# alshai/rowbowt

Hardware: AMD Instinct MI355X
Metric: reads/s (100 bp, count+locate) (higher is better)
Workload: dtype u32/u64

## Files before the change

### rowbowt_amd/csrc/k_runs.hip

```cpp
#include <type_traits>

#include "rbg_runs2_device.hpp"
#include "rbg_jump.h"

namespace rbg {
namespace {

struct PackedBits {
    const uint4 *__restrict__ cp;
    uint4 w;
    uint32_t widx, navail;
    uint64_t sr;
    __device__ __forceinline__ uint32_t next_word() {
        if (widx == 4) { w = *cp++; widx = 0; }
        const uint32_t v = w.x;
        w.x = w.y; w.y = w.z; w.z = w.w;
        ++widx;
        return v;
    }
    __device__ __forceinline__ uint32_t take(uint32_t nb) {
        if (navail < nb) { sr |= static_cast<uint64_t>(next_word()) << navail; navail += 32; }
        const uint32_t v = static_cast<uint32_t>(sr & ((uint64_t(1) << nb) - 1));
        sr >>= nb;
        navail -= nb;
        return v;
    }
};

struct JumpLoad {
    const uint4 *__restrict__ tab;
    __device__ __forceinline__ void operator()(uint64_t b, uint32_t s, uint32_t kw[4], uint32_t vw[4]) const {
        const uint4 *sl = tab + (4 * b + 2 * s);
        const uint4 k = sl[0], v = sl[1];
        kw[0] = k.x; kw[1] = k.y; kw[2] = k.z; kw[3] = k.w;
        vw[0] = v.x; vw[1] = v.y; vw[2] = v.z; vw[3] = v.w;
    }
};

template <typename P, bool TOEHOLD, bool PACKED = false, bool STATS = false, bool GLDS = false, bool STAGE = false>
__global__ __launch_bounds__(512, STATS ? 2 : 4) void k_find_range_runs(const DevIndex ix, const void *__restrict__ src_a,
                                                        const void *__restrict__ src_b, const uint64_t N,
                                                        uint64_t *__restrict__ lo_out, uint64_t *__restrict__ hi_out,
                                                        uint64_t *__restrict__ ss_out, unsigned long long *__restrict__ stats,
                                                        const uint32_t *__restrict__ sel, const uint32_t *__restrict__ nsel) {
    const uint64_t Neff = sel ? static_cast<uint64_t>(*nsel) : N;
    const uint8_t *__restrict__ seqs = static_cast<const uint8_t *>(src_a);
    const uint64_t *__restrict__ off = static_cast<const uint64_t *>(src_b);
    const uint4 *__restrict__ chunks = static_cast<const uint4 *>(src_a);
    const uint2 *__restrict__ meta = static_cast<const uint2 *>(src_b);
    __shared__ uint8_t s_lut[256];
    __shared__ uint8_t s_lut2[256];
    __shared__ uint8_t s_mslot[4];
    __shared__ __align__(16) unsigned char s_tile[GLDS ? 8 * kTileBytes : 16];
    __shared__ uint32_t s_codes[STAGE ? 8 * kStageWords * 64 : 1];
    for (int t = threadIdx.x; t < 256; t += blockDim.x) {
        s_lut[t] = ix.lut[t];
        s_lut2[t] = ix.nmajor ? ix.lut2[t] : 0xFFu;
    }
    RBG_RUN_SEARCH2_SHARED;
    const RunSearch2<P> S2 = stage_run_search2<P>(ix, s_tab_first, s_ent2, s_dir2, s_rec2, s_dyn);
    const uint32_t *tab_first = s_tab_first;
    lds_byte *tile = (lds_byte *)s_tile + (GLDS ? (threadIdx.x >> 6) * kTileBytes : 0u);
    if (PACKED || STAGE) {
        for (int t = threadIdx.x; t < 256; t += blockDim.x)
            if (s_lut2[t] != 0xFFu) s_mslot[s_lut2[t] & 3u] = s_lut[t];
        __syncthreads();
    }
    const uint32_t D = ix.run_ksteps, DMASK = ix.run_depth_mask | 1u;
    const uint32_t M = ix.nmajor;
    const uint32_t lane = threadIdx.x & (kWave - 1);
    lds_u32 *codes = (lds_u32 *)s_codes + (STAGE ? (threadIdx.x >> 6) * (kStageWords * 64u) + lane : 0u);
    const StageTab stage_tab{ix.stage_code[0], ix.stage_code[1], ix.stage_byte[0], ix.stage_byte[1], ix.stage_shift};
    const bool stage_on = STAGE && ix.stage_ok != 0 && M == 4;

    unsigned long long c_occ = 0, c_reads = 0;
    uint32_t c_matched = 0;
    unsigned long long st[kStatSearchN] = {0, 0, 0, 0, 0, 0, 0, 0};
    const uint64_t stride = static_cast<uint64_t>(gridDim.x) * blockDim.x;
    const uint64_t wave_first = static_cast<uint64_t>(blockIdx.x) * blockDim.x + (threadIdx.x & ~(kWave - 1));
    for (uint64_t base = wave_first; base < Neff; base += stride) {
        bool valid = base + lane < Neff;
        const uint64_t i = (sel && valid) ? static_cast<uint64_t>(sel[base + lane]) : base + lane;
        uint64_t beg = 0, p = 0;
        PackedBits bs{chunks, make_uint4(0, 0, 0, 0), 4u, 0u, 0ull};
        if (PACKED) {
            if (valid) {
                const uint2 mt = meta[i];
                if (mt.y & 0x80000000u) valid = false;
                else { p = mt.y; bs.cp = chunks + mt.x; }
            }
        } else if (valid) { beg = off[i]; p = off[i + 1]; }
        bool staged = false;
        if constexpr (STAGE && !PACKED) {
            if (stage_on && __ballot(valid && p - beg > kStageCap) == 0) {
                uint32_t nch = 0;
                const bool bad = valid && stage_read(reinterpret_cast<const uint4 *>(seqs), beg, p, stage_tab, codes, nch);
                if (STATS) st[kStChunks] += nch;
                staged = __ballot(bad) == 0;
                if (staged) { p -= beg; beg = 0; }
                else if (STATS) st[kStChunks] -= nch;
            }
        }
        auto walk = [&](auto staged_tag) __attribute__((always_inline)) {
            constexpr bool STAGED = decltype(staged_tag)::value;
            const uint64_t p_end = p;
            uint64_t p_min = p;
            const uint32_t m32 = static_cast<uint32_t>(p);
            uint64_t lo = 0, hi = ix.n - 1;
            uint64_t k = TOEHOLD ? ix.last_run_sample : 0;
            bool alive = valid;
            bool pend = false;
            uint32_t pend_d = 0, pend_rec = 0;
            uint64_t pend_e = 0;
            ByteCursor rd{reinterpret_cast<const uint4 *>(seqs), ~uint64_t(0), make_uint4(0, 0, 0, 0)};
            bool jumped = false;
            if constexpr (STAGED && sizeof(P) == 4) {
                if (valid && ix.jump && m32 >= ix.jump_k) {
                    JumpKey key{{codes[0], codes[64], codes[128], codes[192]}};
                    jump_key_mask(key, ix.jump_k);
                    uint32_t v[3] = {0, 0, 0}, nbk = 0;
                    if (jump_probe(JumpLoad{static_cast<const uint4 *>(ix.jump)}, ix.jump_buckets, key, v, nbk)) {
                        lo = v[0]; hi = v[1];
                        if (TOEHOLD) k = v[2] == 0xFFFFFFFFu ? ~uint64_t(0) : static_cast<uint64_t>(v[2]);
                        p -= ix.jump_k;
                        jumped = true;
                        if (STATS) st[kStSymbols] += ix.jump_k;
                    }
                    if (STATS) st[kStFtab] += nbk;
                }
            }
            if (!jumped && valid && ix.ftab_k && p - beg >= ix.ftab_k) {
                uint64_t idx = 0;
                bool all_major = true;
                PackedBits probe = bs;
                if constexpr (STAGED) {
                    const uint32_t w0 = codes[0];
                    idx = ix.ftab_k >= 16u ? w0 : (w0 & ((1u << (2u * ix.ftab_k)) - 1u));
                } else if (PACKED) {
                    idx = probe.take(2 * ix.ftab_k);
                } else {
                    uint64_t pw = 1;
                    for (uint32_t t = 1; t <= ix.ftab_k; ++t) {
                        const uint32_t mm = s_lut2[rd.at(p - t)];
                        all_major = all_major && mm != 0xFFu;
                        idx += (mm & 3u) * pw;
                        pw *= M;
                    }
                }
                uint64_t flo, fhi2, fk;
                if (STATS) { if (!STAGED) p_min = p - ix.ftab_k; if (all_major) st[kStFtab] += 1; }
                if (all_major && ftab_lookup<P>(ix, idx, flo, fhi2, fk)) {
                    if (PACKED) bs = probe;
                    lo = flo; hi = fhi2;
                    if (TOEHOLD) k = fk;
                    p -= ix.ftab_k;
                    if (STATS) st[kStSymbols] += ix.ftab_k;
                    if (hi < lo) { alive = false; p = beg; }
                }
            }
            struct Pick { uint32_t d, adv, rec; bool ok; };
            auto pick_at = [&](const uint64_t pp) __attribute__((always_inline)) -> Pick {
                Pick s{0u, 1u, 0u, true};
                if constexpr (STAGED) {
                    s.adv = pp < D ? static_cast<uint32_t>(pp) : D;
                    s.adv = 32u - static_cast<uint32_t>(__clz(DMASK & ((2u << (s.adv - 1)) - 1u)));
                    const uint32_t t0 = m32 - static_cast<uint32_t>(pp);
                    const lds_u32 *cw = codes + (t0 >> 4) * 64u;
                    const uint32_t v = __builtin_amdgcn_alignbit(cw[64], cw[0], (t0 & 15u) * 2u) & ((1u << (2u * s.adv)) - 1u);
                    s.rec = run_record(tab_first, s.adv, s.adv == 1 ? static_cast<uint32_t>(s_mslot[v]) : v);
                    s.d = s.adv - 1;
                } else if (PACKED) {
                    s.adv = pp < D ? static_cast<uint32_t>(pp) : D;
                    s.adv = 32u - static_cast<uint32_t>(__clz(DMASK & ((2u << (s.adv - 1)) - 1u)));
                    const uint32_t v = bs.take(2 * s.adv);
                    s.rec = run_record(tab_first, s.adv, s.adv == 1 ? static_cast<uint32_t>(s_mslot[v]) : v);
                    s.d = s.adv - 1;
                } else {
                    const uint64_t q = pp - 1;
                    const uint32_t c = rd.at(q);
                    if (STATS && q < p_min) p_min = q;
                    const uint32_t m0 = s_lut2[c];
                    uint32_t acc = m0;
                    if (m0 != 0xFFu) {
                        uint32_t pw = M, run_acc = m0;
    #pragma unroll 1
                        for (uint32_t t = 1; t < static_cast<uint32_t>(kMaxRunDepth); ++t) {
                            if (t >= D || q < beg + t) break;
                            const uint32_t mm = s_lut2[rd.at(q - t)];
                            if (STATS && q - t < p_min) p_min = q - t;
                            if (mm == 0xFFu) break;
                            run_acc += mm * pw;
                            pw *= M;
                            if ((DMASK >> t) & 1u) { s.adv = t + 1; acc = run_acc; }
                        }
                    }
                    if (s.adv == 1) {
                        const uint32_t slot = s_lut[c];
                        if (slot == 0xFFu || slot >= static_cast<uint32_t>(kLdsSyms)) s.ok = false;
                        else s.rec = run_record(tab_first, 1u, slot);
                    } else {
                        s.d = s.adv - 1;
                        s.rec = run_record(tab_first, s.adv, acc);
                    }
                }
                return s;
            };
            constexpr bool AHEAD = !PACKED || STAGED;
            Pick cur{0u, 1u, 0u, false};
            RunHot Rcur{0, 0};
            if (AHEAD && alive && p > beg) {
                cur = pick_at(p);
                if (cur.ok) Rcur = load_run_tab<P>(S2, cur.d, cur.rec);
            }
            while (__ballot(alive && p > beg)) {
                bool stepping = alive && p > beg;
                if (!AHEAD && stepping) {
                    cur = pick_at(p);
                    if (cur.ok) Rcur = load_run_tab<P>(S2, cur.d, cur.rec);
                }
                if (stepping && !cur.ok) { alive = false; stepping = false; }
                const uint32_t d = cur.d, adv = cur.adv, rec = cur.rec;
                const RunHot R = Rcur;
                const uint64_t p_next = p - adv;
                if (AHEAD && stepping && p_next > beg) {
                    cur = pick_at(p_next);
                    if (cur.ok) Rcur = load_run_tab<P>(S2, cur.d, cur.rec);
                }
                RunStep r;
                lane_lf2_quad<P, STATS, false, GLDS>(S2, stepping, d, rec, R, lo, hi + 1, r, st, tile);
                if (stepping) {
                    if (STATS) st[kStSymbols] += adv;
                    const uint64_t c_inside = r.c_upto - r.c_before;
                    if (c_inside == 0) {
                        alive = false;
                    } else {
                        if (TOEHOLD) {
                            if (r.inside) k = k - adv;
                            else { pend = true; pend_d = d; pend_rec = rec; pend_e = r.samp_e; k = 0; }
                        }
                        lo = r.F + r.c_before;
                        hi = lo + c_inside - 1;
                        p = p_next;
                    }
                }
            }
            if (TOEHOLD && alive && pend) {
                k += run_step_sample2<P>(ix, S2, pend_d, pend_rec, pend_e);
                if (STATS) st[kStResample] += 1;
            }
            if (STATS && !PACKED && !STAGED && p_end > p_min) st[kStChunks] += ((p_end - 1) >> 4) - (p_min >> 4) + 1;
            if (STATS && PACKED && valid) st[kStChunks] += (p_end + 63) >> 6;
            if (!alive) { lo = 1; hi = 0; k = 0; }
            if (valid) {
                lo_out[i] = lo;
                hi_out[i] = hi;
                if (TOEHOLD) ss_out[i] = k;
                c_reads += 1;
                if (alive) { c_matched += 1; c_occ += hi - lo + 1; }
            }
        };
        if (STAGE && staged) walk(std::integral_constant<bool, STAGE>{}); else walk(std::false_type{});
    }
    c_reads = wave_sum(c_reads);
    const unsigned long long w_matched = wave_sum(static_cast<unsigned long long>(c_matched));
    c_occ = wave_sum(c_occ);
    if (lane == 0 && c_reads) {
        atomicAdd(&ix.counters[0], c_reads);
        if (w_matched) atomicAdd(&ix.counters[1], w_matched);
        if (c_occ) atomicAdd(&ix.counters[2], c_occ);
    }
    if (STATS) {
#pragma unroll
        for (int t = 0; t < kStatSearchN; ++t) {
            const unsigned long long v = wave_sum(st[t]);
            if (lane == 0 && v) atomicAdd(&stats[t], v);
        }
    }
}

template <typename P> struct ChunkR { static constexpr int v = 8; };
__device__ __forceinline__ uint64_t locus_toehold_r(const DevIndex &ix, const uint64_t key, const uint64_t *__restrict__ k, const uint64_t i) {
    if (key == ~uint64_t(0)) return k[i];
    const uint32_t low = ix.order_lowbits, db = ix.order_dbits;
    const uint64_t doc = (key >> low) & ((uint64_t(1) << db) - 1u);
    return ix.order_docs[doc] + (((key >> (db + low)) << low) | (key & ((uint64_t(1) << low) - 1u)));
}

template <typename P, typename OUT = uint64_t, bool STATS = false, bool SUB = false, bool HI8 = false>
__global__ __launch_bounds__(256, 4) void k_locate_fill_runs2(const DevIndex ix, const uint64_t *__restrict__ lo,
                                                          const uint64_t *__restrict__ hi, const uint64_t *__restrict__ k,
                                                          const uint64_t N, const uint64_t max_hits,
                                                          const uint64_t *__restrict__ loc_off, OUT *__restrict__ locs,
                                                          const uint64_t *__restrict__ sub, const uint32_t *__restrict__ order,
                                                          const uint64_t *__restrict__ skeys, unsigned long long *__restrict__ stats) {
    constexpr int kChunkR = ChunkR<P>::v;
    constexpr bool RING = true;
    using Stage = ChainStage<P, kChunkR, SUB, RING, HI8>;
    __shared__ Stage S;
    const uint64_t out_elem0 = reinterpret_cast<uintptr_t>(locs) / sizeof(OUT);
    const int wv = threadIdx.x >> 6, lane = threadIdx.x & (kWave - 1);
    unsigned long long c_locs = 0;
    unsigned long long st_phi = 0, st_ent = 0, st_chains = 0;
    const uint64_t n = ix.n;
    const uint64_t stride = static_cast<uint64_t>(gridDim.x) * blockDim.x;
    for (uint64_t base = static_cast<uint64_t>(blockIdx.x) * blockDim.x + wv * kWave; base < N; base += stride) {
        const uint64_t j = base + lane;
        uint64_t i = j;
        if (order && j < N) i = order[j];
        uint64_t occ = 0, k1 = 0, dst = 0;
        if (i < N && j < N) {
            dst = loc_off[i];
            if (skeys) {
                if (ix.order_docs) k1 = locus_toehold_r(ix, skeys[j], k, i);
                else if (sizeof(P) == 4) { const uint32_t k32 = reinterpret_cast<const uint32_t *>(skeys)[j]; k1 = k32 == 0xFFFFFFFFu ? k[i] : k32; }
                else k1 = skeys[j];
                occ = loc_off[i + 1] - dst;
            } else {
                const uint64_t l = lo[i], h = hi[i];
                occ = h >= l ? h - l + 1 : 0;
                if (occ > max_hits) occ = max_hits;
                k1 = k[i];
            }
        }
        const uint64_t minus = (SUB && i < N && j < N) ? sub[i] : 0;
        const uint32_t a = (RING && occ) ? static_cast<uint32_t>((out_elem0 + dst) & static_cast<uint64_t>(kChunkR - 1)) : 0u;
        S.dst[wv][lane] = dst - a;
        if (SUB) S.minus[wv][lane] = minus;
        const bool off_text = Stage::kSentinel && k1 >= n;
        if (off_text && occ) locs[dst] = static_cast<OUT>(k1 - minus);
        c_locs += occ;
        if (STATS && occ) st_chains += 1;
        uint64_t wmax = occ + a;
#pragma unroll
        for (int o = kWave / 2; o > 0; o >>= 1) {
            const uint64_t other = __shfl_xor(wmax, o, kWave);
            wmax = other > wmax ? other : wmax;
        }
        for (uint64_t t0 = 0; t0 < wmax; t0 += kChunkR) {
            const uint32_t cnt = chain_round_count<kChunkR>(occ, t0);
            S.bounds[wv][lane] = chain_window_bounds<kChunkR>(occ, a, t0);
#pragma unroll 1
            for (int e = 0; e < kChunkR; ++e) {
                const bool mine = static_cast<uint32_t>(e) < cnt;
                if (mine && (e || t0)) {
                    uint64_t s;
                    if (k1 >= n) {
                        s = (ix.phi_last_base + (k1 - ix.phi_last_pos)) % n;
                    } else {
                        bool found;
                        uint64_t val;
                        uint32_t ents, rounds;
                        lane_phi<P>(ix, k1, found, val, ents, rounds);
                        if (STATS) { st_phi += 1; st_ent += ents + 7u * rounds; }
                        s = found ? val : ix.phi_last_base + k1 + 1;
                        if (s >= n) s -= n;
                    }
                    k1 = s;
                }
                if (mine) chain_put(S, wv, lane, a + static_cast<uint32_t>(t0) + e, k1, e == 0 && t0 == 0 && off_text);
            }
            wave_lds_sync();
            chain_flush(S, wv, lane, t0, locs);
            wave_lds_sync();
        }
        wave_lds_sync();
    }
    c_locs = wave_sum(c_locs);
    if (lane == 0 && c_locs) atomicAdd(&ix.counters[3], c_locs);
    if (STATS) {
        st_phi = wave_sum(st_phi);
        st_ent = wave_sum(st_ent);
        st_chains = wave_sum(st_chains);
        if (lane == 0) {
            if (st_phi) atomicAdd(&stats[kLsPhiSteps], st_phi);
            if (st_ent) atomicAdd(&stats[kLsPhiOvf], st_ent);
            if (st_chains) atomicAdd(&stats[kLsChains], st_chains);
            if (c_locs) atomicAdd(&stats[kLsLocs], c_locs);
        }
    }
}

}

int launch_find_range_runs_impl(const DevIndex &ix, const LaunchCfg &cfg, const void *src_a, const void *src_b, uint64_t N,
                                uint64_t *lo, uint64_t *hi, uint64_t *ssamp, void *stream, bool packed, unsigned long long *stats,
                                const uint32_t *sel = nullptr, const uint32_t *nsel = nullptr) {
    if (N == 0) return 0;
    hipStream_t st = static_cast<hipStream_t>(stream);
    const size_t lds = run_search2_lds(ix);
    static const bool glds = [] { const char *e = std::getenv("RBG_REC_FETCH"); return !(e && std::strcmp(e, "quad") == 0); }();
    static const bool stage = [] { const char *e = std::getenv("RBG_STAGE_READS"); return !(e && e[0] == '0'); }();
    LaunchCfg c = cfg;
    c.block_threads = 512;
    c.max_blocks = cfg.max_blocks > 0 ? std::max(1, cfg.max_blocks / 2) : 256 * 16;
    const dim3 grid(sel ? std::min(grid_for(c, N), 256) : grid_for(c, N)), block(512);
#define RBG_LAUNCH_FRR1(PT, TOE, PK, STS, GL, SG)                                                      \
    do {                                                                                               \
        auto kern = k_find_range_runs<PT, TOE, PK, STS, GL, SG>;                                       \
        raise_lds(kern, lds, (GL ? 8 * kTileBytes : 0) + (SG ? 8 * kStageWaveBytes : 0));             \
        hipLaunchKernelGGL(kern, grid, block, lds, st, ix, src_a, src_b, N, lo, hi, ssamp, stats, sel, nsel);     \
    } while (0)
#define RBG_LAUNCH_FRR(PT, TOE, PK, STS)                                                               \
    do {                                                                                               \
        if (glds && stage && !PK && !sel) RBG_LAUNCH_FRR1(PT, TOE, false, STS, true, true);            \
        else if (glds) RBG_LAUNCH_FRR1(PT, TOE, PK, STS, true, false);                                 \
        else RBG_LAUNCH_FRR1(PT, TOE, PK, STS, false, false);                                          \
    } while (0)
#define RBG_LAUNCH_FRR2(PT, TOE)                                                                       \
    do {                                                                                               \
        if (stats) { if (packed) return static_cast<int>(hipErrorNotSupported); RBG_LAUNCH_FRR(PT, TOE, false, true); } \
        else if (packed) RBG_LAUNCH_FRR(PT, TOE, true, false);                                         \
        else RBG_LAUNCH_FRR(PT, TOE, false, false);                                                    \
    } while (0)
    if (ix.pos_bytes == 4) {
        if (ssamp) RBG_LAUNCH_FRR2(uint32_t, true); else RBG_LAUNCH_FRR2(uint32_t, false);
    } else {
        if (ssamp) RBG_LAUNCH_FRR2(uint64_t, true); else RBG_LAUNCH_FRR2(uint64_t, false);
    }
#undef RBG_LAUNCH_FRR2
#undef RBG_LAUNCH_FRR
#undef RBG_LAUNCH_FRR1
    return static_cast<int>(hipGetLastError());
}

int launch_find_range_runs(const DevIndex &ix, const LaunchCfg &cfg, const uint8_t *seqs, const uint64_t *off, uint64_t N,
                           uint64_t *lo, uint64_t *hi, uint64_t *ssamp, void *stream, unsigned long long *stats) {
    return launch_find_range_runs_impl(ix, cfg, seqs, off, N, lo, hi, ssamp, stream, false, stats);
}

int launch_find_range_runs_sel(const DevIndex &ix, const LaunchCfg &cfg, const uint8_t *seqs, const uint64_t *off, uint64_t N, uint64_t *lo,
                               uint64_t *hi, uint64_t *ssamp, const uint32_t *sel, const uint32_t *nsel, void *stream) {
    return launch_find_range_runs_impl(ix, cfg, seqs, off, N, lo, hi, ssamp, stream, false, nullptr, sel, nsel);
}

int launch_find_range_runs_packed(const DevIndex &ix, const LaunchCfg &cfg, const uint2 *meta, const uint4 *chunks, uint64_t N,
                                  uint64_t *lo, uint64_t *hi, uint64_t *ssamp, void *stream) {
    return launch_find_range_runs_impl(ix, cfg, chunks, meta, N, lo, hi, ssamp, stream, true, nullptr);
}

int launch_locate_fill_runs(const DevIndex &ix, const LaunchCfg &cfg, const uint64_t *lo, const uint64_t *hi, const uint64_t *k,
                            uint64_t N, uint64_t max_hits, const uint64_t *loc_off, uint64_t *locs, const uint64_t *sub,
                            const void *order, const uint64_t *skeys, void *stream, unsigned long long *stats, uint32_t *locs32) {
    if (N == 0) return 0;
    if ((stats || locs32) && sub) return static_cast<int>(hipErrorInvalidValue);
    hipStream_t st = static_cast<hipStream_t>(stream);
    const dim3 grid(grid_for(cfg, N)), block(256);
    const uint32_t *perm = static_cast<const uint32_t *>(order);
    const bool hi8 = ix.pos_bytes == 8 && ix.n < kChainHi8Limit && chain_hi8_enabled();
#define RBG_LAUNCH_LFR2(PT, OUT, STS, SB, DST) \
    do { \
        if (sizeof(PT) == 8 && hi8) hipLaunchKernelGGL((k_locate_fill_runs2<PT, OUT, STS, SB, sizeof(PT) == 8>), grid, block, 0, st, ix, lo, hi, k, N, max_hits, loc_off, DST, sub, perm, skeys, stats); \
        else hipLaunchKernelGGL((k_locate_fill_runs2<PT, OUT, STS, SB, false>), grid, block, 0, st, ix, lo, hi, k, N, max_hits, loc_off, DST, sub, perm, skeys, stats); \
    } while (0)
    if (locs32) {
        if (ix.pos_bytes != 4) return static_cast<int>(hipErrorInvalidValue);
        RBG_LAUNCH_LFR2(uint32_t, uint32_t, false, false, locs32);
    } else if (stats) {
        if (ix.pos_bytes == 4) RBG_LAUNCH_LFR2(uint32_t, uint64_t, true, false, locs); else RBG_LAUNCH_LFR2(uint64_t, uint64_t, true, false, locs);
    } else if (sub) {
        if (ix.pos_bytes == 4) RBG_LAUNCH_LFR2(uint32_t, uint64_t, false, true, locs); else RBG_LAUNCH_LFR2(uint64_t, uint64_t, false, true, locs);
    } else if (ix.pos_bytes == 4) {
        RBG_LAUNCH_LFR2(uint32_t, uint64_t, false, false, locs);
    } else {
        RBG_LAUNCH_LFR2(uint64_t, uint64_t, false, false, locs);
    }
#undef RBG_LAUNCH_LFR2
    return static_cast<int>(hipGetLastError());
}

}
```

### rowbowt_amd/csrc/rbg_jump.h

```cpp
#pragma once

#include <cstdint>

#if defined(__HIPCC__)
#define RBG_JUMP_HD __host__ __device__ __forceinline__
#else
#define RBG_JUMP_HD inline
#endif

namespace rbg {

constexpr uint32_t kJumpMaxK = 64;
constexpr uint32_t kJumpMinK = 16;
constexpr uint32_t kJumpSlotWords = 8;
constexpr uint32_t kJumpBucketBytes = 64;
constexpr uint32_t kJumpEmptyTag = 0, kJumpFullTag = 1;
constexpr uint32_t kJumpDefaultK = 60;
constexpr uint64_t kJumpAutoMinBytes = uint64_t(256) << 20;

struct JumpKey {
    uint32_t w[4];
};

RBG_JUMP_HD void jump_key_mask(JumpKey &key, uint32_t K) {
    for (uint32_t i = 0; i < 4; ++i) {
        const uint32_t lo_sym = 16u * i;
        const uint32_t keep = K <= lo_sym ? 0u : (K - lo_sym >= 16u ? 16u : K - lo_sym);
        key.w[i] = keep == 16u ? key.w[i] : (key.w[i] & ((1u << (2u * keep)) - 1u));
    }
}

RBG_JUMP_HD void jump_key_set(JumpKey &key, uint32_t t, uint32_t c) {
    key.w[t >> 4] |= (c & 3u) << (2u * (t & 15u));
}

RBG_JUMP_HD uint64_t jump_hash(const JumpKey &key) {
    const uint64_t a = key.w[0] | (static_cast<uint64_t>(key.w[1]) << 32);
    const uint64_t b = key.w[2] | (static_cast<uint64_t>(key.w[3]) << 32);
    uint64_t h = (a * 0x9E3779B97F4A7C15ull) ^ ((b + 0x632BE59BD9B4E019ull) * 0xC2B2AE3D27D4EB4Full);
    h ^= h >> 29;
    h *= 0xBF58476D1CE4E5B9ull;
    h ^= h >> 32;
    return h;
}

RBG_JUMP_HD uint64_t jump_home(uint64_t h, uint64_t nb) {
    return ((h >> 32) * nb) >> 32;
}

template <typename Load>
RBG_JUMP_HD bool jump_probe(const Load &load, uint64_t nb, const JumpKey &key, uint32_t v[3], uint32_t &buckets) {
    uint64_t b = jump_home(jump_hash(key), nb);
    for (uint64_t step = 0; step < nb; ++step) {
        ++buckets;
        for (uint32_t s = 0; s < 2; ++s) {
            uint32_t kw[4], vw[4];
            load(b, s, kw, vw);
            if (vw[3] == kJumpEmptyTag) return false;
            if (kw[0] == key.w[0] && kw[1] == key.w[1] && kw[2] == key.w[2] && kw[3] == key.w[3]) {
                v[0] = vw[0]; v[1] = vw[1]; v[2] = vw[2];
                return true;
            }
        }
        b = b + 1 == nb ? 0 : b + 1;
    }
    return false;
}

inline uint64_t jump_buckets_for(uint64_t keys) { return keys ? keys : 1; }

}
```

Measured before the change: 1.988 billion.

## Fetch jump-table buckets through wave LDS tile with wave-uniform probe loop

Replaces the per-lane direct global loads of jump hash-table slots with a wave-cooperative global-to-LDS fetch of the whole 64-byte bucket. Each lane then reads its bucket back from the LDS tile. The probe loop becomes ballot-driven, so all lanes take part in each fetch round, and the slot-check logic is made branchless in a shared jump_bucket helper. The aim is better-coalesced, wider memory transactions for the random bucket reads. In exchange it adds full vmcnt/lgkmcnt waits per round and makes idle lanes issue loads. It also requires the GLDS template path (a static_assert) whenever STAGED is set.

```diff
diff --git a/rowbowt_amd/csrc/k_runs.hip b/rowbowt_amd/csrc/k_runs.hip
--- a/rowbowt_amd/csrc/k_runs.hip
+++ b/rowbowt_amd/csrc/k_runs.hip
@@ -27,15 +27,27 @@
     }
 };
 
-struct JumpLoad {
-    const uint4 *__restrict__ tab;
-    __device__ __forceinline__ void operator()(uint64_t b, uint32_t s, uint32_t kw[4], uint32_t vw[4]) const {
-        const uint4 *sl = tab + (4 * b + 2 * s);
-        const uint4 k = sl[0], v = sl[1];
-        kw[0] = k.x; kw[1] = k.y; kw[2] = k.z; kw[3] = k.w;
-        vw[0] = v.x; vw[1] = v.y; vw[2] = v.z; vw[3] = v.w;
-    }
-};
+template <bool GLDS>
+__device__ __forceinline__ void jump_fetch(const void *tab, const bool on, const uint64_t b, lds_byte *tile, uint32_t (&bw)[16]) {
+    static_assert(GLDS, "the jump probe fetches through the wave's LDS tile");
+    const uint64_t a = reinterpret_cast<uint64_t>(tab) + (on ? b * kJumpBucketBytes : 0u);
+    u32x4 t0, t1, t2, t3;
+    {
+        const uint32_t a_lo = static_cast<uint32_t>(a), a_hi = static_cast<uint32_t>(a >> 32), p = threadIdx.x & 3u;
+        glds_round<0>(a_lo, a_hi, p, tile);
+        glds_round<1>(a_lo, a_hi, p, tile);
+        glds_round<2>(a_lo, a_hi, p, tile);
+        glds_round<3>(a_lo, a_hi, p, tile);
+        asm volatile("s_waitcnt vmcnt(0)" ::: "memory");
+        const lds_byte *own = tile + (threadIdx.x & 3u) * kTileRound + (threadIdx.x & 60u) * 16u;
+        typedef __attribute__((address_space(3))) const u32x4 lds_u32x4;
+        t0 = reinterpret_cast<lds_u32x4 *>(own)[0]; t1 = reinterpret_cast<lds_u32x4 *>(own)[1];
+        t2 = reinterpret_cast<lds_u32x4 *>(own)[2]; t3 = reinterpret_cast<lds_u32x4 *>(own)[3];
+        asm volatile("s_waitcnt lgkmcnt(0)" ::: "memory");
+    }
+    bw[0] = t0.x; bw[1] = t0.y; bw[2] = t0.z; bw[3] = t0.w; bw[4] = t1.x; bw[5] = t1.y; bw[6] = t1.z; bw[7] = t1.w;
+    bw[8] = t2.x; bw[9] = t2.y; bw[10] = t2.z; bw[11] = t2.w; bw[12] = t3.x; bw[13] = t3.y; bw[14] = t3.z; bw[15] = t3.w;
+}
 
 template <typename P, bool TOEHOLD, bool PACKED = false, bool STATS = false, bool GLDS = false, bool STAGE = false>
 __global__ __launch_bounds__(512, STATS ? 2 : 4) void k_find_range_runs(const DevIndex ix, const void *__restrict__ src_a,
@@ -115,15 +127,28 @@
             ByteCursor rd{reinterpret_cast<const uint4 *>(seqs), ~uint64_t(0), make_uint4(0, 0, 0, 0)};
             bool jumped = false;
             if constexpr (STAGED && sizeof(P) == 4) {
-                if (valid && ix.jump && m32 >= ix.jump_k) {
+                bool probing = valid && ix.jump && m32 >= ix.jump_k;
+                if (__ballot(probing)) {
                     JumpKey key{{codes[0], codes[64], codes[128], codes[192]}};
                     jump_key_mask(key, ix.jump_k);
+                    const uint64_t nb = ix.jump_buckets;
+                    uint64_t b = jump_home(jump_hash(key), nb);
                     uint32_t v[3] = {0, 0, 0}, nbk = 0;
-                    if (jump_probe(JumpLoad{static_cast<const uint4 *>(ix.jump)}, ix.jump_buckets, key, v, nbk)) {
+                    do {
+                        uint32_t bw[16];
+                        jump_fetch<GLDS>(ix.jump, probing, b, tile, bw);
+                        if (probing) {
+                            ++nbk;
+                            const uint32_t r = jump_bucket(bw, key, v);
+                            jumped = r == kJumpHit;
+                            probing = r == kJumpNext && nbk < nb;
+                            b = jump_next(b, nb);
+                        }
+                    } while (__ballot(probing));
+                    if (jumped) {
                         lo = v[0]; hi = v[1];
                         if (TOEHOLD) k = v[2] == 0xFFFFFFFFu ? ~uint64_t(0) : static_cast<uint64_t>(v[2]);
                         p -= ix.jump_k;
-                        jumped = true;
                         if (STATS) st[kStSymbols] += ix.jump_k;
                     }
                     if (STATS) st[kStFtab] += nbk;
diff --git a/rowbowt_amd/csrc/rbg_jump.h b/rowbowt_amd/csrc/rbg_jump.h
--- a/rowbowt_amd/csrc/rbg_jump.h
+++ b/rowbowt_amd/csrc/rbg_jump.h
@@ -48,21 +48,31 @@
     return ((h >> 32) * nb) >> 32;
 }
 
+constexpr uint32_t kJumpNext = 0, kJumpHit = 1, kJumpAbsent = 2;
+RBG_JUMP_HD uint32_t jump_bucket(const uint32_t bw[16], const JumpKey &key, uint32_t v[3]) {
+    const bool f0 = bw[7] != kJumpEmptyTag, f1 = bw[15] != kJumpEmptyTag;
+    const bool m0 = f0 && bw[0] == key.w[0] && bw[1] == key.w[1] && bw[2] == key.w[2] && bw[3] == key.w[3];
+    const bool m1 = f0 && f1 && bw[8] == key.w[0] && bw[9] == key.w[1] && bw[10] == key.w[2] && bw[11] == key.w[3];
+    const bool hit = m0 || m1;
+    v[0] = hit ? (m0 ? bw[4] : bw[12]) : v[0];
+    v[1] = hit ? (m0 ? bw[5] : bw[13]) : v[1];
+    v[2] = hit ? (m0 ? bw[6] : bw[14]) : v[2];
+    return hit ? kJumpHit : (f0 && f1 ? kJumpNext : kJumpAbsent);
+}
+
+RBG_JUMP_HD uint64_t jump_next(uint64_t b, uint64_t nb) { return b + 1 == nb ? 0 : b + 1; }
+
 template <typename Load>
 RBG_JUMP_HD bool jump_probe(const Load &load, uint64_t nb, const JumpKey &key, uint32_t v[3], uint32_t &buckets) {
     uint64_t b = jump_home(jump_hash(key), nb);
     for (uint64_t step = 0; step < nb; ++step) {
         ++buckets;
-        for (uint32_t s = 0; s < 2; ++s) {
-            uint32_t kw[4], vw[4];
-            load(b, s, kw, vw);
-            if (vw[3] == kJumpEmptyTag) return false;
-            if (kw[0] == key.w[0] && kw[1] == key.w[1] && kw[2] == key.w[2] && kw[3] == key.w[3]) {
-                v[0] = vw[0]; v[1] = vw[1]; v[2] = vw[2];
-                return true;
-            }
-        }
-        b = b + 1 == nb ? 0 : b + 1;
+        uint32_t bw[16];
+        load(b, 0u, bw, bw + 4);
+        load(b, 1u, bw + 8, bw + 12);
+        const uint32_t r = jump_bucket(bw, key, v);
+        if (r != kJumpNext) return r == kJumpHit;
+        b = jump_next(b, nb);
     }
     return false;
 }
```

New measurement: 2.083 billion (median of 6 runs). 1.05x the previous value.
